# PeihaoChen/RSPNet

Hardware: AMD Instinct MI355X
Metric: clips/sec pretext step (c3d 16x112x112, B=32/GPU) (higher is better)
Workload: dtype f32

## Files before the change

### include/rspnet_hip.h

```cpp
#ifndef RSPNET_HIP_H
#define RSPNET_HIP_H

#include <stddef.h>
#include <stdint.h>

#ifdef __cplusplus
extern "C" {
#endif

#define RSP_OK 0
#define RSP_EINVAL (-1)
#define RSP_EWORKSPACE (-2)
#define RSP_ELAUNCH (-3)
#define RSP_EUNSUPPORTED (-4)

const char* rsp_strerror(int code);
const char* rsp_last_error(void);
const char* rsp_last_conv_kernel(void);
int rsp_version(void);

typedef struct rsp_conv3d_desc {
  int32_t N, Di, Hi, Wi, Cin;
  int32_t Do, Ho, Wo, Cout;
  int32_t kT, kH, kW;
// ... 70 lines not shown
  int32_t kT, kH, kW, sT, sH, sW, pT, pH, pW;
  int32_t in_ld, out_ld, res_ld;
} rsp_pool3d_desc;

int rsp_bn_act_pool_fwd(const rsp_pool3d_desc* d, const float* y, const float* scale_shift, const float* residual,
                        int relu, const float* gate, float* out, void* stream);

int rsp_bn_act_maxpool_applicable(const rsp_pool3d_desc* d);
int rsp_bn_act_maxpool_fwd(const rsp_pool3d_desc* d, const float* y, const float* scale_shift, int relu, const float* gate, float* out,
                           int32_t* argmax, void* stream);

size_t rsp_bn_bwd_workspace(const rsp_pool3d_desc* d);
int rsp_bn_act_pool_bwd(const rsp_pool3d_desc* d, const float* y, const float* residual, const float* dout,
                        const float* gamma, const float* mean_invstd, const float* scale_shift, int relu, float* dy,
                        float* dres, float* dgamma, float* dbeta, int32_t c_valid, const float* gate, const float* dmean,
                        void* workspace, size_t workspace_bytes, void* stream);

int rsp_bn_act_pool_sel_applicable(const rsp_pool3d_desc* d);
int rsp_bn_act_pool_sel_fwd(const rsp_pool3d_desc* d, const float* y, const float* scale_shift, int relu, float* out, float* y_sel,
                            void* stream);
int rsp_bn_act_pool_sel_bwd(const rsp_pool3d_desc* d, const float* y, const float* y_sel, const float* dout, const float* gamma,
                            const float* mean_invstd, const float* scale_shift, int relu, float* dy, float* dgamma, float* dbeta,
                            int32_t c_valid, void* workspace, size_t workspace_bytes, void* stream);

int rsp_bn_act_minmax_fwd(const float* y_max, const float* y_min, int64_t positions, int32_t C, int32_t out_ld,
                          const float* scale_shift, int relu, float* out, void* stream);

size_t rsp_bn_eval_bwd_workspace(const rsp_pool3d_desc* d);
int rsp_bn_eval_act_pool_bwd(const rsp_pool3d_desc* d, const float* y, const float* residual, const float* dout,
                             const float* mean_invstd, const float* scale_shift, int relu, float* dy, float* dres,
                             float* dgamma, float* dbeta, int32_t c_valid, void* workspace, size_t workspace_bytes,
                             void* stream);

int rsp_maxpool3d_fwd(const rsp_pool3d_desc* d, const float* x, float* out, int32_t* argmax, void* stream);
int rsp_maxpool3d_bwd(const rsp_pool3d_desc* d, const float* dout, const int32_t* argmax, float* dx, void* stream);

size_t rsp_gate_fwd_workspace(int32_t N, int32_t P, int32_t C);
int rsp_gate_fwd(const float* x, int32_t N, int32_t P, int32_t C, int32_t in_ld, const float* w, const float* b,
                 float* out, int32_t out_ld, float* mean, float* gate, void* workspace, size_t workspace_bytes,
                 void* stream);
int rsp_bn_gate_sums(const float* y, int32_t N, int32_t P, int32_t C, int32_t y_ld, const float* scale_shift, int relu,
                     float* act, int32_t act_ld, const float* w, const float* b, float* mean, float* gate, void* workspace,
                     size_t workspace_bytes, void* stream);
int rsp_gate_apply(const float* x, int32_t N, int32_t P, int32_t C, int32_t in_ld, const float* gate, float* out, int32_t out_ld,
                   void* stream);
int rsp_gate_bwd_params(const float* y, const float* scale_shift, int relu, const float* dout, int32_t N, int32_t P, int32_t C,
// ... 146 lines not shown
```

### rspnet_amd/_lib.py

```python
from __future__ import annotations

import ctypes as C
import os
from typing import Optional

_HERE = os.path.dirname(os.path.abspath(__file__))
LIB_PATH = os.environ.get("RSPNET_HIP_LIB") or os.path.join(_HERE, "librspnet_hip.so")

c_f32p = C.c_void_p
c_i32p = C.c_void_p
c_stream = C.c_void_p


class ConvDesc(C.Structure):
    _fields_ = [(n, C.c_int32) for n in (
        "N", "Di", "Hi", "Wi", "Cin", "Do", "Ho", "Wo", "Cout", "kT", "kH", "kW", "sT", "sH", "sW",
        "pT", "pH", "pW", "in_ld", "out_ld")]


class PoolDesc(C.Structure):
    _fields_ = [(n, C.c_int32) for n in (
        "N", "Di", "Hi", "Wi", "C", "Do", "Ho", "Wo", "kT", "kH", "kW", "sT", "sH", "sW", "pT", "pH", "pW",
        "in_ld", "out_ld", "res_ld")]

# ... 43 lines not shown
SIGNATURES = {
    "rsp_strerror": (C.c_char_p, [C.c_int]),
    "rsp_last_error": (C.c_char_p, []),
    "rsp_last_conv_kernel": (C.c_char_p, []),
    "rsp_version": (C.c_int, []),
    "rsp_conv3d_packed_fwd_elems": (_sz, [_PD]),
    "rsp_conv3d_pack_fwd": (C.c_int, [_PD, _p, _p, _p]),
    "rsp_conv3d_stat_tiles": (_i32, [_PD]),
    "rsp_conv3d_fwd_workspace": (_sz, [_PD]),
    "rsp_conv3d_fwd": (C.c_int, [_PD, _p, _p, _p, _p, _p, _p, _sz, _p]),
    "rsp_conv3d_stem_pooled_applicable": (C.c_int, [_PD]),
    "rsp_conv3d_stem_pooled_fwd": (C.c_int, [_PD, _p, _p, _p, _p, _p, _p, _p]),
    "rsp_conv3d_dgrad_workspace": (_sz, [_PD]),
    "rsp_conv3d_dgrad": (C.c_int, [_PD, _p, _p, _p, _p, _sz, _p]),
    "rsp_conv3d_packed_dgrad_elems": (_sz, [_PD]),
    "rsp_conv3d_dgrad_packed": (C.c_int, [_PD, _p, _p, _p, _p, _sz, _p]),
    "rsp_conv3d_pack_jobs": (_i32, [_PD, _i32, _i32, _i32, _p, _p, _p, _i32]),
    "rsp_pack_run": (C.c_int, [_p, _i32, _i32, _p]),
    "rsp_conv3d_pack_forget": (None, [_p]),
    "rsp_conv3d_wgrad_workspace": (_sz, [_PD]),
    "rsp_conv3d_rowgeom_bytes": (_sz, [_PD]),
    "rsp_conv3d_rowgeom": (C.c_int, [_PD, _p, _p]),
    "rsp_conv3d_wgrad": (C.c_int, [_PD, _p, _p, _p, _p, _i32, _i32, _p, _p, _sz, _p]),
    "rsp_conv3d_kernel_name": (C.c_char_p, [_PD, C.c_int]),
    "rsp_conv3d_executed_fraction": (C.c_double, [_PD, C.c_int]),
    "rsp_conv3d_set_option": (C.c_int, [C.c_char_p, _i32]),
    "rsp_fastdiv_check": (C.c_int, [C.c_int, C.c_int]),
    "rsp_bn_finalize_workspace": (_sz, [_i32, _i32]),
    "rsp_bn_finalize": (C.c_int, [_p, _i32, _i32, _i32, _i32, _i64, _p, _p, _p, _f, _f, _p, _p, _p, _p, _p, _p, _sz, _p]),
    "rsp_bn_running_update": (C.c_int, [_p, _i32, _i32, _p]),
    "rsp_bn_act_pool_fwd": (C.c_int, [_PP, _p, _p, _p, C.c_int, _p, _p, _p]),
    "rsp_bn_act_maxpool_applicable": (C.c_int, [_PP]),
    "rsp_bn_act_maxpool_fwd": (C.c_int, [_PP, _p, _p, C.c_int, _p, _p, _p, _p]),
    "rsp_bn_bwd_workspace": (_sz, [_PP]),
    "rsp_bn_act_pool_bwd": (C.c_int, [_PP, _p, _p, _p, _p, _p, _p, C.c_int, _p, _p, _p, _p, _i32, _p, _p, _p, _sz, _p]),
    "rsp_bn_act_pool_sel_applicable": (C.c_int, [_PP]),
    "rsp_bn_act_pool_sel_fwd": (C.c_int, [_PP, _p, _p, C.c_int, _p, _p, _p]),
    "rsp_bn_act_pool_sel_bwd": (C.c_int, [_PP, _p, _p, _p, _p, _p, _p, C.c_int, _p, _p, _p, _i32, _p, _sz, _p]),
    "rsp_bn_act_minmax_fwd": (C.c_int, [_p, _p, _i64, _i32, _i32, _p, C.c_int, _p, _p]),
    "rsp_bn_eval_bwd_workspace": (_sz, [_PP]),
    "rsp_bn_eval_act_pool_bwd": (C.c_int, [_PP, _p, _p, _p, _p, _p, C.c_int, _p, _p, _p, _p, _i32, _p, _sz, _p]),
    "rsp_maxpool3d_fwd": (C.c_int, [_PP, _p, _p, _p, _p]),
    "rsp_maxpool3d_bwd": (C.c_int, [_PP, _p, _p, _p, _p]),
    "rsp_gate_fwd_workspace": (_sz, [_i32, _i32, _i32]),
    "rsp_gate_fwd": (C.c_int, [_p, _i32, _i32, _i32, _i32, _p, _p, _p, _i32, _p, _p, _p, _sz, _p]),
    "rsp_bn_gate_sums": (C.c_int, [_p, _i32, _i32, _i32, _i32, _p, C.c_int, _p, _i32, _p, _p, _p, _p, _p, _sz, _p]),
# ... 109 lines not shown
```

### rspnet_amd/csrc/bn_pool.hip

```cpp
#include "common.h"

namespace {

__global__ __launch_bounds__(256) void bn_finalize_stage1(const float* __restrict__ part, int tiles, int C, int ld, int S,
                                                          double* __restrict__ out) {
  __shared__ double red[4][64][2];
  const int c = blockIdx.x * 64 + (threadIdx.x & 63);
  const int rl = threadIdx.x >> 6;
  const int per = (tiles + S - 1) / S;
  const int t0 = blockIdx.y * per, t1 = min(tiles, t0 + per);
  double s = 0.0, ss = 0.0;
  if (c < C)
    for (int t = t0 + rl; t < t1; t += 4) {
      const float2 v = *reinterpret_cast<const float2*>(part + ((long long)t * ld + c) * 2);
      s += (double)v.x;
      ss += (double)v.y;
    }
  red[rl][threadIdx.x & 63][0] = s;
  red[rl][threadIdx.x & 63][1] = ss;
  __syncthreads();
  if (rl == 0 && c < C) {
    const int l = threadIdx.x;
    out[((long long)blockIdx.y * C + c) * 2 + 0] = red[0][l][0] + red[1][l][0] + red[2][l][0] + red[3][l][0];
    out[((long long)blockIdx.y * C + c) * 2 + 1] = red[0][l][1] + red[1][l][1] + red[2][l][1] + red[3][l][1];
// ... 845 lines not shown
      constexpr int NW = MODE == 2 ? 4 : 8;
      long long off[NW];
      window_offsets<NW>(d, off);
      for (; o < o_end; o += stride) {
        const int op = (int)o;
        const int q1 = fastdiv(op, p.dWo), ow = op - q1 * d.Wo;
        const int q2 = fastdiv(q1, p.dHo), oh = q1 - q2 * d.Ho;
        const int n = fastdiv(q2, p.dDo), od = q2 - n * d.Do;
        const long long base = (((long long)n * d.Di + od * d.sT) * d.Hi + oh * d.sH) * d.Wi + ow * d.sW;
        float yv[NW][VEC], r[NW][VEC], g[VEC], best[VEC];
        int bi[VEC];
#pragma unroll
        for (int w = 0; w < NW; ++w) {
          load_vec<VEC>(p.y + (base + off[w]) * d.in_ld + c, yv[w]);
          if (p.res) load_vec<VEC>(p.res + (base + off[w]) * d.res_ld + c, r[w]);
        }
        load_vec<VEC>(p.dout + o * d.out_ld + c, g);
#pragma unroll
        for (int e = 0; e < VEC; ++e) { best[e] = -INFINITY; bi[e] = 0; }
#pragma unroll
        for (int w = 0; w < NW; ++w)
#pragma unroll
          for (int e = 0; e < VEC; ++e) {
            float z = fmaf(yv[w][e], sc[e], sh[e]);
            if (p.res) z += r[w][e];
            const float v = p.relu ? rsp_relu(z) : z;
            if (rsp_max_takes(v, best[e])) { best[e] = v; bi[e] = w; }
          }
#pragma unroll
        for (int w = 0; w < NW; ++w) {
          float ov[VEC], dz[VEC];
#pragma unroll
          for (int e = 0; e < VEC; ++e) {
            dz[e] = (bi[e] == w && !(p.relu && rsp_relu_blocks(best[e]))) ? g[e] : 0.f;
            const float xhat = (yv[w][e] - mean[e]) * invstd[e];
            ov[e] = gam[e] * invstd[e] * (dz[e] - m1[e] - xhat * m2[e]);
          }
          store_vec<VEC>(p.dy + (base + off[w]) * d.in_ld + c, ov);
          if (p.dres) store_vec<VEC>(p.dres + (base + off[w]) * d.res_ld + c, dz);
        }
      }
    }
    return;
  }
  for (; o < o_end; o += stride) {
    float g[VEC];
    load_vec<VEC>(p.dout + o * d.out_ld + c, g);
    if (MODE == 1 || nwin == 1) {
      if (p.gate) gated_grad<VEC>(p, fastdiv(fastdiv(fastdiv((int)o, p.dWo), p.dHo), p.dDo), c, g);
      float yv[VEC], z[VEC], ov[VEC], dz[VEC];
      zval<VEC>(p, o, c, sc, sh, yv, z);
#pragma unroll
      for (int e = 0; e < VEC; ++e) {
        dz[e] = (p.relu && rsp_relu_blocks(z[e])) ? 0.f : g[e];
        const float xhat = (yv[e] - mean[e]) * invstd[e];
        ov[e] = gam[e] * invstd[e] * (dz[e] - m1[e] - xhat * m2[e]);
      }
      store_vec<VEC>(p.dy + o * d.in_ld + c, ov);
      if (p.dres) store_vec<VEC>(p.dres + o * d.res_ld + c, dz);
// ... 424 lines not shown
      (!gate || rsp_aligned16(gate)))
    return rsp_bn_act_maxpool_fwd(d, y, scale_shift, relu, gate, out, nullptr, stream);
  PoolParams p;
  p.d = *d; p.y = y; p.ss = scale_shift; p.res = residual; p.gate = gate; p.out = out; p.relu = relu;
  const bool vec = d->C % 4 == 0 && d->in_ld % 4 == 0 && d->out_ld % 4 == 0 && rsp_aligned16(y) && rsp_aligned16(out) &&
                   rsp_aligned16(scale_shift) && (!residual || (d->res_ld % 4 == 0 && rsp_aligned16(residual))) &&
                   (!gate || rsp_aligned16(gate));
  p.cg = vec ? d->C / 4 : d->C;
  const Layout L = make_layout(d, p.cg, 4);
  RSP_REQUIRE(L.npos < (1ll << 31), "rsp_bn_act_pool_fwd: more than 2^31 - 1 output positions");
  set_layout(p, L);
  RSP_BN_LAUNCH(bn_act_pool_fwd_kernel, vec, bn_mode(d, gate != nullptr), L.grid, (hipStream_t)stream, p);
  return rsp_check_launch("bn_act_pool_fwd_kernel");
}

size_t rsp_bn_bwd_workspace(const rsp_pool3d_desc* d) {
  if (!pool_ok(d, true)) return 0;
  return rsp_align_up((size_t)2048 * d->C * 2 * sizeof(float), 256) + (size_t)d->C * 2 * sizeof(double);
}

static int bn_act_pool_bwd(const rsp_pool3d_desc* d, const float* y, const float* y_sel, const float* residual, const float* dout,
                           const float* gamma, const float* mean_invstd, const float* scale_shift, int relu, float* dy,
                           float* dres, float* dgamma, float* dbeta, int32_t c_valid, const float* gate, const float* dmean,
                           void* workspace, size_t workspace_bytes, void* stream) {
  RSP_REQUIRE(pool_ok(d, true), "rsp_bn_act_pool_bwd: needs disjoint windows (kernel == stride, no padding)");
  RSP_REQUIRE(!gate || (dmean && d->kT * d->kH * d->kW == 1 && d->sT * d->sH * d->sW == 1 && !residual),
              "rsp_bn_act_pool_bwd: a gated unit has a unit window, no residual, and needs dmean");
  RSP_REQUIRE(c_valid > 0 && c_valid <= d->C, "rsp_bn_act_pool_bwd: bad valid channel count");
  RSP_REQUIRE(y && dout && mean_invstd && scale_shift && dy && workspace, "rsp_bn_act_pool_bwd: null pointer");
  if (workspace_bytes < rsp_bn_bwd_workspace(d)) {
    rsp_set_error("rsp_bn_act_pool_bwd: workspace too small");
    return RSP_EWORKSPACE;
  }
  hipStream_t s = (hipStream_t)stream;
  BwdParams p;
  memset(&p, 0, sizeof p);
  p.d = *d; p.y = y; p.res = residual; p.dout = dout; p.gamma = gamma; p.mi = mean_invstd; p.ss = scale_shift;
  p.dy = dy; p.dres = dres; p.relu = relu;
  p.Cv = c_valid;
  p.gate = gate; p.dmean = dmean;
  p.invP = 1.f / (float)((long long)d->Di * d->Hi * d->Wi);
  p.count = (long long)d->N * d->Di * d->Hi * d->Wi;
  const bool vec = d->C % 4 == 0 && d->in_ld % 4 == 0 && d->out_ld % 4 == 0 && rsp_aligned16(y) && rsp_aligned16(dout) &&
                   rsp_aligned16(dy) && rsp_aligned16(scale_shift) && rsp_aligned16(mean_invstd) &&
                   (!gamma || c_valid != d->C || rsp_aligned16(gamma)) &&
                   (!residual || (d->res_ld % 4 == 0 && rsp_aligned16(residual) && (!dres || rsp_aligned16(dres)))) &&
                   (!gate || (rsp_aligned16(gate) && rsp_aligned16(dmean)));
  p.cg = vec ? d->C / 4 : d->C;
  p.partial = reinterpret_cast<float*>(workspace);
  double* sums = reinterpret_cast<double*>(reinterpret_cast<unsigned char*>(workspace) +
                                           rsp_align_up((size_t)2048 * d->C * 2 * sizeof(float), 256));
  p.sums = sums;
  const Layout L = make_layout(d, p.cg, 4);
  RSP_REQUIRE(L.npos < (1ll << 31), "rsp_bn_act_pool_bwd: more than 2^31 - 1 output positions");
  set_layout(p, L);
  p.nblocks = reduce_blocks(d, p.cg);
  dim3 rgrid(p.nblocks, rsp_cdiv(p.cg, 256));
  const int mode = bn_mode(d, gate != nullptr);
  if (y_sel) {
    RSP_REQUIRE(vec && (mode == 2 || mode == 3) && !residual && rsp_aligned16(y_sel),
                "rsp_bn_act_pool_sel_bwd: y_sel needs what rsp_bn_act_pool_sel_fwd needs, and no residual");
    p.ysel = y_sel;
    hipLaunchKernelGGL(bn_bwd_reduce_sel_kernel<4>, rgrid, dim3(256), 0, s, p);
  } else {
    RSP_BN_LAUNCH(bn_bwd_reduce_kernel, vec, mode, rgrid, s, p);
  }
  int rc = rsp_check_launch("bn_bwd_reduce_kernel");
  if (rc != RSP_OK) return rc;
  hipLaunchKernelGGL(bn_bwd_finalize_kernel, dim3(rsp_cdiv(d->C, FIN_CH)), dim3(1024), 0, s, p.partial, p.nblocks, d->C, c_valid, sums,
                     dgamma, dbeta);
  rc = rsp_check_launch("bn_bwd_finalize_kernel");
  if (rc != RSP_OK) return rc;
  const bool exact = d->Di % d->sT == 0 && d->Hi % d->sH == 0 && d->Wi % d->sW == 0 && d->kT * d->kH * d->kW <= 8;
  if (exact) {
    RSP_BN_LAUNCH(bn_bwd_apply_win_kernel, vec, mode, L.grid, s, p);
    return rsp_check_launch("bn_bwd_apply_win_kernel");
  }
  const long long total = (long long)d->N * d->Di * d->Hi * d->Wi * p.cg;
  if (vec) hipLaunchKernelGGL(bn_bwd_apply_kernel<4>, dim3(grid_for(total)), dim3(256), 0, s, p);
  else hipLaunchKernelGGL(bn_bwd_apply_kernel<1>, dim3(grid_for(total)), dim3(256), 0, s, p);
  return rsp_check_launch("bn_bwd_apply_kernel");
}

int rsp_bn_act_pool_bwd(const rsp_pool3d_desc* d, const float* y, const float* residual, const float* dout,
                        const float* gamma, const float* mean_invstd, const float* scale_shift, int relu, float* dy,
                        float* dres, float* dgamma, float* dbeta, int32_t c_valid, const float* gate, const float* dmean,
                        void* workspace, size_t workspace_bytes, void* stream) {
  return bn_act_pool_bwd(d, y, nullptr, residual, dout, gamma, mean_invstd, scale_shift, relu, dy, dres, dgamma, dbeta, c_valid, gate,
                         dmean, workspace, workspace_bytes, stream);
}

int rsp_bn_act_pool_sel_bwd(const rsp_pool3d_desc* d, const float* y, const float* y_sel, const float* dout, const float* gamma,
                            const float* mean_invstd, const float* scale_shift, int relu, float* dy, float* dgamma, float* dbeta,
                            int32_t c_valid, void* workspace, size_t workspace_bytes, void* stream) {
  RSP_REQUIRE(y_sel, "rsp_bn_act_pool_sel_bwd: null pointer");
  return bn_act_pool_bwd(d, y, y_sel, nullptr, dout, gamma, mean_invstd, scale_shift, relu, dy, nullptr, dgamma, dbeta, c_valid, nullptr,
                         nullptr, workspace, workspace_bytes, stream);
}

static int eval_bwd_mode(const rsp_pool3d_desc* d) {
  const int m = bn_mode(d, false);
  if (m == 1) return 1;
  const bool exact = d->Di % d->sT == 0 && d->Hi % d->sH == 0 && d->Wi % d->sW == 0;
  return exact ? m : 0;
}

static long long eval_bwd_npos(const rsp_pool3d_desc* d, int mode) {
  if (mode != 0) return (long long)d->N * d->Do * d->Ho * d->Wo;
  return (long long)d->N * rsp_cdiv(d->Di, d->sT) * rsp_cdiv(d->Hi, d->sH) * rsp_cdiv(d->Wi, d->sW);
}

size_t rsp_bn_eval_bwd_workspace(const rsp_pool3d_desc* d) {
  if (!pool_ok(d, true)) return 0;
  const long long npos = eval_bwd_npos(d, eval_bwd_mode(d));
  const long long rows = npos < EVAL_BWD_MAX_BLOCKS ? npos : EVAL_BWD_MAX_BLOCKS;
  return (size_t)rows * d->C * 2 * sizeof(float);
}

#define RSP_BN_EVAL_LAUNCH_S(V, M, grid, stream, p)                                                                       \
  do {                                                                                                                    \
    if (sums) hipLaunchKernelGGL((bn_eval_bwd_kernel<V, M, true>), grid, dim3(256), 0, stream, p);                        \
// ... 60 lines not shown
```

### rspnet_amd/csrc/conv_stem.h

```cpp
#pragma once
#include "common.h"

bool rsp_conv_desc_ok(const rsp_conv3d_desc* d);
bool rsp_stem_applicable(const rsp_conv3d_desc* d);
int rsp_stem_tiles(const rsp_conv3d_desc* d);
size_t rsp_stem_packed_elems(const rsp_conv3d_desc* d);
int rsp_stem_pack(const rsp_conv3d_desc* d, const float* w_ref, float* w_packed, hipStream_t s);
int rsp_stem_fwd(const rsp_conv3d_desc* d, const float* x, const float* w_packed, const float* bias, float* y,
                 float* stat_partials, hipStream_t s);
const char* rsp_stem_kernel_name(const rsp_conv3d_desc* d);
bool rsp_stem_pooled_applicable(const rsp_conv3d_desc* d);
int rsp_stem_pooled_fwd(const rsp_conv3d_desc* d, const float* x, const float* w_packed, const float* bias, float* y_max, float* y_min,
                        float* stat_partials, hipStream_t s);
void rsp_stem_note_packed(const void* w_packed, bool three_channels);
void rsp_stem_forget_packed(const void* w_packed);
const char* rsp_wgrad_kernel_name(const rsp_conv3d_desc* d);
double rsp_wgrad_executed_fraction(const rsp_conv3d_desc* d);
```

### rspnet_amd/csrc/conv_stem.hip

```cpp
#include "conv_stem.h"

#include <mutex>
#include <unordered_map>

namespace {

struct StemParams {
  const float* __restrict__ x;
  const float* __restrict__ w;
  const float* __restrict__ bias;
  float* __restrict__ y;
  float* __restrict__ stat;
  int N, Di, Hi, Wi, Do, Ho, Wo;
  int kT, kH, kW, sT, sH, sW, pT, pH, pW;
  int Cout, out_ld;
  int tw_shift;
  int HT, WT, WTh, WTL;
  int npix, npix_r;
  int FR;
  int ntaps, nchunks;
  int tiles_h, tiles_w, tiles;
  unsigned x_bytes, w_bytes;
  int wide;
  float* __restrict__ ymax;
// ... 395 lines not shown
      }
      s += __shfl_xor(s, 32);
      ss += __shfl_xor(ss, 32);
      if (h == 0) {
        red[(wave * 64 + col) * 2 + 0] = s;
        red[(wave * 64 + col) * 2 + 1] = ss;
      }
    }
    if (p.stat) {
      __syncthreads();
      if (t < 64 && t < p.Cout) {
        float s = 0.f, ss = 0.f;
#pragma unroll
        for (int w = 0; w < 4; ++w) {
          s += red[(w * 64 + t) * 2 + 0];
          ss += red[(w * 64 + t) * 2 + 1];
        }
        float* o = p.stat + ((long long)tile * p.Cout + t) * 2;
        o[0] = s;
        o[1] = ss;
      }
    }
    cur ^= 1;
  }
}

__global__ void stem_pack_kernel(const float* __restrict__ w, float* __restrict__ out, int Cout, int kT, int kH, int kW,
                                 int ntaps, long long total) {
  for (long long i = blockIdx.x * (long long)blockDim.x + threadIdx.x; i < total; i += (long long)gridDim.x * blockDim.x) {
    const int ci = (int)(i & 3), n = (int)((i >> 2) & 63), tap = (int)(i >> 8);
    float v = 0.f;
    if (tap < ntaps && n < Cout) {
      const int kw = tap % kW, r = tap / kW;
      const int kh = r % kH, kt = r / kH;
      v = w[((((long long)n * 4 + ci) * kT + kt) * kH + kh) * kW + kw];
    }
    out[i] = v;
  }
}

struct StemPlan {
  bool ok;
  int G, TCH, nchunks, tw_shift, HT, WT, WTh, WTL, npix, npix_r, FR, tiles_h, tiles_w;
  bool resident;
  bool wide_ok;
  long long tiles;
// ... 187 lines not shown
}

bool rsp_stem_pooled_applicable(const rsp_conv3d_desc* d) { return stem_pooled_ok(d, stem_plan(d)); }

int rsp_stem_pooled_fwd(const rsp_conv3d_desc* d, const float* x, const float* w_packed, const float* bias, float* y_max, float* y_min,
                        float* stat_partials, hipStream_t stream) {
  const StemPlan pl = stem_plan(d);
  RSP_REQUIRE(stem_pooled_ok(d, pl), "rsp_conv3d_stem_pooled_fwd: descriptor not covered (rsp_conv3d_stem_pooled_applicable)");
  RSP_REQUIRE(rsp_aligned16(x) && rsp_aligned16(w_packed) && rsp_aligned16(y_max) && rsp_aligned16(y_min),
              "rsp_conv3d_stem_pooled_fwd: input, packed weight and both outputs must be 16-byte aligned");
  StemParams p = stem_params(d, pl, x, w_packed, bias, stat_partials);
  p.ymax = y_max; p.ymin = y_min; p.pool_ld = d->Cout;
  if (stem_three_channels(w_packed)) {
    switch (pl.G) {
      case 7: return launch_stem_pooled<7, 3>(p, pl, stream);
      default: return launch_stem_pooled<5, 3>(p, pl, stream);
    }
  }
  switch (pl.G) {
    case 7: return launch_stem_pooled<7, 4>(p, pl, stream);
    default: return launch_stem_pooled<5, 4>(p, pl, stream);
  }
}
```

### rspnet_amd/engine.py

```python
from __future__ import annotations

import contextlib
import os
from dataclasses import dataclass, field
from typing import Dict, List, NamedTuple, Optional, Tuple, Union

import torch
from torch import nn

from . import ops as _ops
from .ops import ConvGeom, PoolGeom

Triple = Tuple[int, int, int]


@dataclass
class ConvBN:
    conv: nn.Module
    bn: nn.Module
    src: int
    dst: int
    k: Triple
    s: Triple = (1, 1, 1)
    p: Triple = (0, 0, 0)
# ... 143 lines not shown

class _CatConv:
    weight: torch.Tensor = None


def _adjacent_cat(ts):
    t0 = ts[0]
    if not all(t.is_contiguous() and t.shape[1:] == t0.shape[1:] and t.dtype == t0.dtype for t in ts):
        return None
    end = t0.data_ptr() + t0.numel() * t0.element_size()
    for t in ts[1:]:
        if t.data_ptr() != end or t.untyped_storage().data_ptr() != t0.untyped_storage().data_ptr():
            return None
        end += t.numel() * t.element_size()
    shape = (sum(t.shape[0] for t in ts),) + tuple(t0.shape[1:])
    stride = tuple(t0.stride())
    return torch.as_strided(t0, shape, stride, t0.storage_offset())


INPUT_CHANNEL_PAD = 4
GATE_BWD_FUSED = not os.environ.get("RSP_NO_GATE_BWD_FUSION")
STEM_POOLED = not os.environ.get("RSP_NO_STEM_POOLED")
BN_BWD_SEL = not os.environ.get("RSP_NO_BN_BWD_SEL")


class VirtualStem:

    def __init__(self, node):
        self.conv = node.conv
        w = node.conv.weight
        Cout, cin, kT, kH, kW = w.shape
        assert cin == 3 and kW == 7 and node.s[2] == 2 and node.p[2] == 3
        self.holders, self.idx, self.src, self.dst = [], [], [], []
        co = torch.arange(Cout).view(Cout, 1, 1, 1, 1)
        c4 = torch.arange(4).view(1, 4, 1, 1, 1)
        kt = torch.arange(kT).view(1, 1, kT, 1, 1)
        kh = torch.arange(kH).view(1, 1, 1, kH, 1)
        j = torch.arange(6).view(1, 1, 1, 1, 6)
        for off in (3, 1):
            r = 4 * j + c4 - off
            valid = ((r >= 0) & (r < 21)).expand(Cout, 4, kT, kH, 6)
            real = ((((co * 3 + r % 3) * kT + kt) * kH + kh) * 7 + torch.div(r, 3, rounding_mode="floor")).expand(Cout, 4, kT, kH, 6)
            idx = torch.where(valid, real, torch.full_like(real, w.numel())).reshape(-1)
            flat_valid = valid.reshape(-1).nonzero().view(-1)
            self.idx.append(idx.to(w.device))
            self.src.append(flat_valid.to(w.device))
# ... 482 lines not shown

    def take_grad(self, node, C):
        return _view(self.dslots[node.into[0]], node.into, C) if node.into is not None else self.dslots.pop(node.dst)

    def issued(self, ni):
        if self.hook is not None:
            self.hook(ni, self.branches.grads_ready)

    def input_grad(self, src, cg, dy, conv):
        if src != self.plan.input_slot or self.want_input_grad:
            self.add_grad(src, self.be.conv_dgrad_packed(cg, dy, self.packed.get_dgrad(conv, cg)))

    def convbn(self, node, ni, key=None):
        key = ni if key is None else key
        sv = self.ctx.saved.pop(key)
        if isinstance(sv, _SavedVStem):
            return self.convbn_virtual(node, sv, ni)
        if sv.gate is not None:
            return self.convbn_gated(node, sv, ni)
        if sv.eval_mode:
            return self.convbn_eval(node, sv, ni)
        bn, grad_of = node.bn, self.grad_of
        dout = self.take_grad(node, sv.cg.Cout)
        sel = {} if sv.y_sel is None else {"y_sel": sv.y_sel}
        dy, dres = self.be.bn_act_pool_bwd(sv.pg, sv.y, sv.res, dout, bn.weight.data, sv.mi, sv.ss, node.relu,
                                           node.residual is not None, grad_of(bn.weight), grad_of(bn.bias), **sel)
        self.convbn_tail(node, sv, ni, dy, dres, True)

    def convbn_virtual(self, node, sv, ni):
        be, grad_of, vs, cg = self.be, self.grad_of, sv.vs, sv.cg
        assert node.src == self.plan.input_slot and not self.want_input_grad, "a virtual-pixel stem reads the clip: no input gradient"
        dout = self.dslots.pop(node.dst)
        bn = node.bn
        dy, _ = be.bn_act_pool_bwd(sv.pg, sv.y, None, dout, bn.weight.data, sv.mi, sv.ss, node.relu, False, grad_of(bn.weight), grad_of(bn.bias))
        gw = grad_of(node.conv.weight)
        if gw is not None:
            N, do, ho, Wo, Cp = dy.shape
            dyv = dy.view(N, do, ho, Wo // 2, 2 * Cp)
            gflat = gw.view(-1)
            gflat.zero_()
            for c, xc in enumerate((sv.x_e, sv.x_o)):
                gv = torch.empty_like(vs.holders[c].weight)
                be.conv_wgrad(cg, xc, dyv[..., c * Cp:(c + 1) * Cp], gv)
                gflat.index_add_(0, vs.dst[c], gv.view(-1).index_select(0, vs.src[c]))
        self.issued(ni)

    def convbn_gated(self, node, sv, ni):
        bn, grad_of, sg = node.bn, self.grad_of, sv.gate
        gnode = self.plan.nodes[sg.at]
        dout = self.take_grad(gnode, sv.cg.Cout)
# ... 99 lines not shown
```

### rspnet_amd/ops.py

```python
from __future__ import annotations

import collections
import contextlib
import ctypes as C
import functools
from dataclasses import dataclass
from typing import Optional, Tuple

import torch

from . import _lib


@dataclass(frozen=True)
class ConvGeom:
    N: int
    Di: int
    Hi: int
    Wi: int
    Cin: int
    Cout: int
    k: Tuple[int, int, int]
    s: Tuple[int, int, int]
    p: Tuple[int, int, int]
# ... 58 lines not shown
@functools.lru_cache(maxsize=4096)
def executed_fraction(g: "ConvGeom", which: int) -> float:
    d = g.desc()
    return float(_lib.load().rsp_conv3d_executed_fraction(C.byref(d), which))


@functools.lru_cache(maxsize=8192)
def _pack_signature(g: "ConvGeom", which: int, cout_src: int, cin_src: int):
    lib = _lib.load()
    d = g.desc()
    buf = (_lib.PackJob * 64)()
    cnt = lib.rsp_conv3d_pack_jobs(C.byref(d), which, cout_src, cin_src, C.c_void_p(1 << 20), C.c_void_p(1 << 30), buf, 64)
    lib.rsp_conv3d_pack_forget(C.c_void_p(1 << 30))
    if cnt < 0:
        _lib.check(cnt, "rsp_conv3d_pack_jobs")
    n = (lib.rsp_conv3d_packed_dgrad_elems if which else lib.rsp_conv3d_packed_fwd_elems)(C.byref(d))
    return (int(n), bytes(buf)[:cnt * C.sizeof(_lib.PackJob)])


@functools.lru_cache(maxsize=4096)
def _stem_pooled_ok(g: "ConvGeom") -> bool:
    d = g.desc()
    return bool(_lib.load().rsp_conv3d_stem_pooled_applicable(C.byref(d)))


@functools.lru_cache(maxsize=4096)
def _pool_plan(pg: "PoolGeom", in_ld, out_ld, res_ld):
    lib = _lib.load()
    d = pg.desc(in_ld=in_ld, out_ld=out_ld, res_ld=res_ld)
    ref = C.byref(d)
    return d, ref, lib.rsp_bn_bwd_workspace(ref), pg.out_dims


def _ptr(t: Optional[torch.Tensor]):
    return None if t is None else C.c_void_p(t.data_ptr())


_raw_stream = getattr(torch._C, "_cuda_getCurrentRawStream", None)
_get_device = getattr(torch._C, "_cuda_getDevice", None)


def _stream():
    if _raw_stream is not None and _get_device is not None:
        return C.c_void_p(_raw_stream(_get_device()))
    return C.c_void_p(torch.cuda.current_stream().cuda_stream)

# ... 322 lines not shown
                        want_dres: bool, dgamma_out, dbeta_out, dy_out=None, y_sel=None):
        in_ld = _rows_ld(y, "y")
        d, dref, wsb, _ = _pool_plan(pg, in_ld, _rows_ld(dout, "dout"), None if residual is None else _rows_ld(residual, "residual"))
        dy = _dy_target(y, in_ld, dy_out)
        dres = torch.empty_like(y) if want_dres else None
        ws = self._workspace(y.device, wsb)
        c_valid = pg.C if gamma is None else int(gamma.shape[0])
        e0 = self._ev()
        n_in = y.numel()
        if y_sel is not None:
            if residual is not None or want_dres:
                raise _lib.RspError("bn_act_pool_bwd: y_sel with a residual")
            _lib.check(self.lib.rsp_bn_act_pool_sel_bwd(dref, _ptr(y), _ptr(_chk(y_sel, "y_sel")), _ptr(dout), _ptr(gamma), _ptr(mean_invstd),
                                                        _ptr(scale_shift), int(relu), _ptr(dy), _ptr(dgamma_out), _ptr(dbeta_out), c_valid,
                                                        _ptr(ws), wsb, _stream()), "rsp_bn_act_pool_sel_bwd")
            self._log_hbm("bn_bwd(reduce+apply)", 4 * (y_sel.numel() + 2 * dout.numel() + 2 * n_in), e0)
            return dy, dres
        _lib.check(self.lib.rsp_bn_act_pool_bwd(dref, _ptr(y), _ptr(residual), _ptr(dout), _ptr(gamma),
                                                _ptr(mean_invstd), _ptr(scale_shift), int(relu), _ptr(dy), _ptr(dres),
                                                _ptr(dgamma_out), _ptr(dbeta_out), c_valid, None, None, _ptr(ws), wsb, _stream()),
                   "rsp_bn_act_pool_bwd")
        self._log_hbm("bn_bwd(reduce+apply)", 4 * (2 * (n_in * (1 if residual is None else 2) + dout.numel()) + n_in * (2 if want_dres else 1)), e0)
        return dy, dres

    def bn_eval_act_pool_bwd(self, pg: PoolGeom, y, residual, dout, mean_invstd, scale_shift, relu: bool, want_dres: bool,
                             dgamma_out, dbeta_out, dy_out=None):
        in_ld = _rows_ld(y, "y")
        d, dref, _, _ = _pool_plan(pg, in_ld, _rows_ld(dout, "dout"), None if residual is None else _rows_ld(residual, "residual"))
        dy = _dy_target(y, in_ld, dy_out)
        if want_dres and residual is None:
            raise _lib.RspError("want_dres without a residual")
        dres = torch.empty(y.shape, dtype=torch.float32, device=y.device) if want_dres else None
        if want_dres and d.res_ld != pg.C:
            raise _lib.RspError("residual: a residual whose gradient is wanted must be contiguous")
        sums = dgamma_out is not None or dbeta_out is not None
        c_valid = pg.C
        for v in (dgamma_out, dbeta_out):
            if v is not None:
                c_valid = int(v.shape[0])
        wsb = int(self.lib.rsp_bn_eval_bwd_workspace(dref)) if sums else 0
        ws = self._workspace(y.device, wsb) if sums else None
        e0 = self._ev()
        _lib.check(self.lib.rsp_bn_eval_act_pool_bwd(dref, _ptr(y), _ptr(residual), _ptr(dout), _ptr(mean_invstd), _ptr(scale_shift),
                                                     int(relu), _ptr(dy), _ptr(dres), _ptr(dgamma_out), _ptr(dbeta_out), c_valid,
                                                     _ptr(ws), wsb, _stream()), "rsp_bn_eval_act_pool_bwd")
        n_in = y.numel()
# ... 532 lines not shown
```

Baseline: 357.2.

## Fuse stem BN/ReLU/maxpool backward apply into the stem weight-gradient kernel

Adds a fused stem backward kernel. It recomputes the BN+ReLU+2x2 maxpool input gradient in registers from y and dout and feeds it straight into MFMA-based weight-gradient accumulation against the input halo staged in LDS. The first-layer dy tensor is never written to or read back from HBM. The BN reduction pass still runs separately, and a small reduce kernel sums the per-block partials. In exchange there is a more specialised code path with strict applicability checks and a recompute of the BN backward maths.

```diff
diff --git a/include/rspnet_hip.h b/include/rspnet_hip.h
--- a/include/rspnet_hip.h
+++ b/include/rspnet_hip.h
@@ -116,6 +116,13 @@
 int rsp_bn_act_pool_sel_bwd(const rsp_pool3d_desc* d, const float* y, const float* y_sel, const float* dout, const float* gamma,
                             const float* mean_invstd, const float* scale_shift, int relu, float* dy, float* dgamma, float* dbeta,
                             int32_t c_valid, void* workspace, size_t workspace_bytes, void* stream);
+
+size_t rsp_conv3d_stem_bn_wgrad_workspace(const rsp_conv3d_desc* d, const rsp_pool3d_desc* pd);
+int rsp_conv3d_stem_bn_wgrad(const rsp_conv3d_desc* d, const rsp_pool3d_desc* pd, const float* x, const float* y, const float* y_sel,
+                             const float* residual, const float* gate, const float* dout, const float* gamma,
+                             const float* mean_invstd, const float* scale_shift, int relu, float* dw_ref, int32_t cout_valid,
+                             int32_t cin_valid, float* dgamma, float* dbeta, int32_t c_valid, void* workspace,
+                             size_t workspace_bytes, void* stream);
 
 int rsp_bn_act_minmax_fwd(const float* y_max, const float* y_min, int64_t positions, int32_t C, int32_t out_ld,
                           const float* scale_shift, int relu, float* out, void* stream);
diff --git a/rspnet_amd/_lib.py b/rspnet_amd/_lib.py
--- a/rspnet_amd/_lib.py
+++ b/rspnet_amd/_lib.py
@@ -89,6 +89,8 @@
     "rsp_conv3d_rowgeom_bytes": (_sz, [_PD]),
     "rsp_conv3d_rowgeom": (C.c_int, [_PD, _p, _p]),
     "rsp_conv3d_wgrad": (C.c_int, [_PD, _p, _p, _p, _p, _i32, _i32, _p, _p, _sz, _p]),
+    "rsp_conv3d_stem_bn_wgrad_workspace": (_sz, [_PD, _PP]),
+    "rsp_conv3d_stem_bn_wgrad": (C.c_int, [_PD, _PP, _p, _p, _p, _p, _p, _p, _p, _p, _p, C.c_int, _p, _i32, _i32, _p, _p, _i32, _p, _sz, _p]),
     "rsp_conv3d_kernel_name": (C.c_char_p, [_PD, C.c_int]),
     "rsp_conv3d_executed_fraction": (C.c_double, [_PD, C.c_int]),
     "rsp_conv3d_set_option": (C.c_int, [C.c_char_p, _i32]),
diff --git a/rspnet_amd/csrc/bn_bwd_math.h b/rspnet_amd/csrc/bn_bwd_math.h
--- /dev/null
+++ b/rspnet_amd/csrc/bn_bwd_math.h
@@ -0,0 +1,17 @@
+#pragma once
+#include "common.h"
+
+__device__ __forceinline__ float rsp_bn_bwd_z(float y, float sc, float sh) { return fmaf(y, sc, sh); }
+
+__device__ __forceinline__ void rsp_bn_bwd_scan(float v, int w, float& best, int& bi) {
+  if (rsp_max_takes(v, best)) { best = v; bi = w; }
+}
+
+__device__ __forceinline__ float rsp_bn_bwd_dz(int w, int bi, float best, bool relu, float g) {
+  return (bi == w && !(relu && rsp_relu_blocks(best))) ? g : 0.f;
+}
+
+__device__ __forceinline__ float rsp_bn_bwd_dy(float y, float dz, float mean, float invstd, float gam, float m1, float m2) {
+  const float xhat = (y - mean) * invstd;
+  return gam * invstd * (dz - m1 - xhat * m2);
+}
diff --git a/rspnet_amd/csrc/bn_pool.hip b/rspnet_amd/csrc/bn_pool.hip
--- a/rspnet_amd/csrc/bn_pool.hip
+++ b/rspnet_amd/csrc/bn_pool.hip
@@ -1,4 +1,6 @@
 #include "common.h"
+#include "bn_bwd_math.h"
+#include "conv_stem.h"
 
 namespace {
 
@@ -891,19 +893,18 @@
         for (int w = 0; w < NW; ++w)
 #pragma unroll
           for (int e = 0; e < VEC; ++e) {
-            float z = fmaf(yv[w][e], sc[e], sh[e]);
+            float z = rsp_bn_bwd_z(yv[w][e], sc[e], sh[e]);
             if (p.res) z += r[w][e];
             const float v = p.relu ? rsp_relu(z) : z;
-            if (rsp_max_takes(v, best[e])) { best[e] = v; bi[e] = w; }
+            rsp_bn_bwd_scan(v, w, best[e], bi[e]);
           }
 #pragma unroll
         for (int w = 0; w < NW; ++w) {
           float ov[VEC], dz[VEC];
 #pragma unroll
           for (int e = 0; e < VEC; ++e) {
-            dz[e] = (bi[e] == w && !(p.relu && rsp_relu_blocks(best[e]))) ? g[e] : 0.f;
-            const float xhat = (yv[w][e] - mean[e]) * invstd[e];
-            ov[e] = gam[e] * invstd[e] * (dz[e] - m1[e] - xhat * m2[e]);
+            dz[e] = rsp_bn_bwd_dz(w, bi[e], best[e], p.relu != 0, g[e]);
+            ov[e] = rsp_bn_bwd_dy(yv[w][e], dz[e], mean[e], invstd[e], gam[e], m1[e], m2[e]);
           }
           store_vec<VEC>(p.dy + (base + off[w]) * d.in_ld + c, ov);
           if (p.dres) store_vec<VEC>(p.dres + (base + off[w]) * d.res_ld + c, dz);
@@ -1374,12 +1375,12 @@
 static int bn_act_pool_bwd(const rsp_pool3d_desc* d, const float* y, const float* y_sel, const float* residual, const float* dout,
                            const float* gamma, const float* mean_invstd, const float* scale_shift, int relu, float* dy,
                            float* dres, float* dgamma, float* dbeta, int32_t c_valid, const float* gate, const float* dmean,
-                           void* workspace, size_t workspace_bytes, void* stream) {
+                           void* workspace, size_t workspace_bytes, void* stream, const double** sums_only = nullptr) {
   RSP_REQUIRE(pool_ok(d, true), "rsp_bn_act_pool_bwd: needs disjoint windows (kernel == stride, no padding)");
   RSP_REQUIRE(!gate || (dmean && d->kT * d->kH * d->kW == 1 && d->sT * d->sH * d->sW == 1 && !residual),
               "rsp_bn_act_pool_bwd: a gated unit has a unit window, no residual, and needs dmean");
   RSP_REQUIRE(c_valid > 0 && c_valid <= d->C, "rsp_bn_act_pool_bwd: bad valid channel count");
-  RSP_REQUIRE(y && dout && mean_invstd && scale_shift && dy && workspace, "rsp_bn_act_pool_bwd: null pointer");
+  RSP_REQUIRE(y && dout && mean_invstd && scale_shift && (dy || sums_only) && workspace, "rsp_bn_act_pool_bwd: null pointer");
   if (workspace_bytes < rsp_bn_bwd_workspace(d)) {
     rsp_set_error("rsp_bn_act_pool_bwd: workspace too small");
     return RSP_EWORKSPACE;
@@ -1423,6 +1424,10 @@
                      dgamma, dbeta);
   rc = rsp_check_launch("bn_bwd_finalize_kernel");
   if (rc != RSP_OK) return rc;
+  if (sums_only) {
+    *sums_only = sums;
+    return RSP_OK;
+  }
   const bool exact = d->Di % d->sT == 0 && d->Hi % d->sH == 0 && d->Wi % d->sW == 0 && d->kT * d->kH * d->kW <= 8;
   if (exact) {
     RSP_BN_LAUNCH(bn_bwd_apply_win_kernel, vec, mode, L.grid, s, p);
@@ -1449,6 +1454,17 @@
   return bn_act_pool_bwd(d, y, y_sel, nullptr, dout, gamma, mean_invstd, scale_shift, relu, dy, nullptr, dgamma, dbeta, c_valid, nullptr,
                          nullptr, workspace, workspace_bytes, stream);
 }
+
+}
+
+int rsp_bn_bwd_sums(const rsp_pool3d_desc* d, const float* y, const float* y_sel, const float* dout, const float* gamma,
+                    const float* mean_invstd, const float* scale_shift, int relu, float* dgamma, float* dbeta, int32_t c_valid,
+                    void* workspace, size_t workspace_bytes, void* stream, const double** sums) {
+  return bn_act_pool_bwd(d, y, y_sel, nullptr, dout, gamma, mean_invstd, scale_shift, relu, nullptr, nullptr, dgamma, dbeta, c_valid, nullptr,
+                         nullptr, workspace, workspace_bytes, stream, sums);
+}
+
+extern "C" {
 
 static int eval_bwd_mode(const rsp_pool3d_desc* d) {
   const int m = bn_mode(d, false);
diff --git a/rspnet_amd/csrc/conv_stem.h b/rspnet_amd/csrc/conv_stem.h
--- a/rspnet_amd/csrc/conv_stem.h
+++ b/rspnet_amd/csrc/conv_stem.h
@@ -14,5 +14,8 @@
                         float* stat_partials, hipStream_t s);
 void rsp_stem_note_packed(const void* w_packed, bool three_channels);
 void rsp_stem_forget_packed(const void* w_packed);
+int rsp_bn_bwd_sums(const rsp_pool3d_desc* d, const float* y, const float* y_sel, const float* dout, const float* gamma,
+                    const float* mean_invstd, const float* scale_shift, int relu, float* dgamma, float* dbeta, int32_t c_valid,
+                    void* workspace, size_t workspace_bytes, void* stream, const double** sums);
 const char* rsp_wgrad_kernel_name(const rsp_conv3d_desc* d);
 double rsp_wgrad_executed_fraction(const rsp_conv3d_desc* d);
diff --git a/rspnet_amd/csrc/conv_stem.hip b/rspnet_amd/csrc/conv_stem.hip
--- a/rspnet_amd/csrc/conv_stem.hip
+++ b/rspnet_amd/csrc/conv_stem.hip
@@ -1,4 +1,5 @@
 #include "conv_stem.h"
+#include "bn_bwd_math.h"
 
 #include <mutex>
 #include <unordered_map>
@@ -441,6 +442,234 @@
       }
     }
     cur ^= 1;
+  }
+}
+
+struct StemBwdParams {
+  StemParams s;
+  const float* __restrict__ yv;
+  const float* __restrict__ dout;
+  const float* __restrict__ ss;
+  const float* __restrict__ mi;
+  const float* __restrict__ gamma;
+  const double* __restrict__ sums;
+  float* __restrict__ partial;
+  int dout_ld, Cv;
+  long long count;
+};
+
+__global__ __launch_bounds__(256, 2) void stem_bn_wgrad_kernel(const StemBwdParams q) {
+  const StemParams& p = q.s;
+  typedef __attribute__((address_space(3))) void* lptr_t;
+  extern __shared__ __attribute__((aligned(16))) unsigned char smem_raw[];
+  const int hsz = p.kT * p.npix_r * 4;
+  float* halo = reinterpret_cast<float*>(smem_raw);
+
+  const int t = threadIdx.x;
+  const int lane = t & 63;
+  const int wave = __builtin_amdgcn_readfirstlane(t >> 6);
+  const int l32 = lane & 31, h = lane >> 5;
+
+  __amdgpu_buffer_rsrc_t rsrc_x = __builtin_amdgcn_make_buffer_rsrc(const_cast<float*>(p.x), 0, (int)p.x_bytes, 0x00020000);
+  int hyy[4], wxp[4];
+#pragma unroll
+  for (int i = 0; i < 4; ++i) {
+    const int k = i * 256 + t;
+    hyy[i] = -(1 << 20);
+    wxp[i] = 0;
+    if (k < p.npix) {
+      hyy[i] = k / p.WTL;
+      wxp[i] = k - hyy[i] * p.WTL;
+    }
+  }
+  auto issue_halo = [&](int tile, int buf) {
+    const int wb = tile % p.tiles_w;
+    int q0 = tile / p.tiles_w;
+    const int hb = q0 % p.tiles_h;
+    q0 /= p.tiles_h;
+    const int to = q0 % p.Do, n = q0 / p.Do;
+    const int hi0 = hb * 8 - p.pH, wi0 = wb * 16 - p.pW;
+    unsigned hrel[4];
+#pragma unroll
+    for (int i = 0; i < 4; ++i) {
+      const int hi = hi0 + hyy[i], wi = wi0 + wxp[i];
+      hrel[i] = ((unsigned)hi < (unsigned)p.Hi && (unsigned)wi < (unsigned)p.Wi) ? (unsigned)((hi * p.Wi + wi) * 16) : 0xffffffffu;
+    }
+    for (int f = 0; f < p.kT; ++f) {
+      const int ti = to - p.pT + f;
+      const bool okf = (unsigned)ti < (unsigned)p.Di;
+      const unsigned fbase = (unsigned)(((long long)(n * p.Di + (okf ? ti : 0)) * p.Hi * p.Wi) * 16);
+#pragma unroll
+      for (int i = 0; i < 4; ++i) {
+        if (i * 256 + wave * 64 < p.npix_r) {
+          const unsigned off = (okf & (hrel[i] != 0xffffffffu)) ? fbase + hrel[i] : 0xffffffffu;
+          float* dst = halo + buf * hsz + (f * p.npix_r + i * 256 + wave * 64) * 4;
+          __builtin_amdgcn_raw_ptr_buffer_load_lds(rsrc_x, (lptr_t)dst, 16, off, 0, 0, 0);
+        }
+      }
+    }
+  };
+
+  float sc[2], sh[2], mean[2], invstd[2], gam[2], m1[2], m2[2];
+  bool cok[2];
+  const double invn = 1.0 / (double)q.count;
+#pragma unroll
+  for (int j = 0; j < 2; ++j) {
+    const int c = 32 * j + l32;
+    cok[j] = c < p.Cout;
+    sc[j] = sh[j] = mean[j] = invstd[j] = gam[j] = m1[j] = m2[j] = 0.f;
+    if (cok[j]) {
+      sc[j] = q.ss[c];
+      sh[j] = q.ss[p.Cout + c];
+      mean[j] = q.mi[c];
+      invstd[j] = q.mi[p.Cout + c];
+      gam[j] = c < q.Cv ? (q.gamma ? q.gamma[c] : 1.f) : 0.f;
+      m1[j] = (float)(q.sums[2 * c] * invn);
+      m2[j] = (float)(q.sums[2 * c + 1] * invn);
+    }
+  }
+  int boff[3];
+#pragma unroll
+  for (int b = 0; b < 3; ++b) {
+    const int n = 32 * b + l32;
+    int off = 0;
+    if (n < 3 * p.ntaps) {
+      const int tap = n / 3, ch = n - 3 * tap;
+      const int kw = tap % p.kW, r = tap / p.kW;
+      const int kh = r % p.kH, kt = r / p.kH;
+      off = ((kt * p.npix_r) + kh * p.WTL + kw) * 16 + ch * 4;
+    }
+    boff[b] = off + (2 * wave * p.WTL + 4 * h) * 16;
+  }
+  const int erow = p.WTL * 16;
+
+  const int HoP = p.Ho >> 1, WoP = p.Wo >> 1;
+  auto load_patch = [&](int tile, float (&yv)[2][16], float (&g)[2][4]) {
+    const int wb = tile % p.tiles_w;
+    int q0 = tile / p.tiles_w;
+    const int hb = q0 % p.tiles_h;
+    q0 /= p.tiles_h;
+    const float* yb = q.yv + (((long long)q0 * p.Ho + hb * 8 + 2 * wave) * p.Wo + wb * 16 + 4 * h) * p.out_ld;
+    const float* gb = q.dout + (((long long)q0 * HoP + hb * 4 + wave) * WoP + wb * 8 + 2 * h) * q.dout_ld;
+#pragma unroll
+    for (int j = 0; j < 2; ++j) {
+      const int c = cok[j] ? 32 * j + l32 : 0;
+#pragma unroll
+      for (int e = 0; e < 16; ++e) {
+        const int ro = (e >> 3) * p.Wo + 8 * ((e >> 2) & 1) + (e & 3);
+        yv[j][e] = yb[(long long)ro * p.out_ld + c];
+      }
+#pragma unroll
+      for (int k = 0; k < 4; ++k) g[j][k] = gb[(long long)((k >> 1) * 4 + (k & 1)) * q.dout_ld + c];
+    }
+  };
+
+  floatx16 acc[2][3];
+#pragma unroll
+  for (int j = 0; j < 2; ++j)
+#pragma unroll
+    for (int b = 0; b < 3; ++b)
+#pragma unroll
+      for (int e = 0; e < 16; ++e) acc[j][b][e] = 0.f;
+
+  float yn[2][16], gn[2][4];
+  int cur = 0;
+  if ((int)blockIdx.x < p.tiles) {
+    load_patch(blockIdx.x, yn, gn);
+    issue_halo(blockIdx.x, 0);
+  }
+  for (int tile = blockIdx.x; tile < p.tiles; tile += gridDim.x) {
+    __syncthreads();
+    const int next = tile + gridDim.x;
+    floatx16 a[2];
+#pragma unroll
+    for (int j = 0; j < 2; ++j)
+#pragma unroll
+      for (int k = 0; k < 4; ++k) {
+        const int el[4] = {2 * k, 2 * k + 1, 2 * k + 8, 2 * k + 9};
+        float yw[4], best = -INFINITY;
+        int bi = 0;
+        const float g = cok[j] ? gn[j][k] : 0.f;
+#pragma unroll
+        for (int w = 0; w < 4; ++w) yw[w] = cok[j] ? yn[j][el[w]] : 0.f;
+#pragma unroll
+        for (int w = 0; w < 4; ++w) rsp_bn_bwd_scan(rsp_relu(rsp_bn_bwd_z(yw[w], sc[j], sh[j])), w, best, bi);
+#pragma unroll
+        for (int w = 0; w < 4; ++w)
+          a[j][el[w]] = rsp_bn_bwd_dy(yw[w], rsp_bn_bwd_dz(w, bi, best, true, g), mean[j], invstd[j], gam[j], m1[j], m2[j]);
+      }
+    const char* bp = reinterpret_cast<const char*>(halo + cur * hsz);
+    auto bval = [&](int e, int b) {
+      return *reinterpret_cast<const float*>(bp + boff[b] + (e >> 3) * erow + (8 * ((e >> 2) & 1) + (e & 3)) * 16);
+    };
+#pragma unroll
+    for (int e = 0; e < 8; ++e) {
+      float bv[3];
+#pragma unroll
+      for (int b = 0; b < 3; ++b) bv[b] = bval(e, b);
+#pragma unroll
+      for (int b = 0; b < 3; ++b)
+#pragma unroll
+        for (int j = 0; j < 2; ++j) acc[j][b] = __builtin_amdgcn_mfma_f32_32x32x2f32(a[j][e], bv[b], acc[j][b], 0, 0, 0);
+    }
+    float bq[8][3];
+#pragma unroll
+    for (int e = 0; e < 8; ++e)
+#pragma unroll
+      for (int b = 0; b < 3; ++b) bq[e][b] = bval(8 + e, b);
+    if (next < p.tiles) {
+      load_patch(next, yn, gn);
+      issue_halo(next, cur ^ 1);
+    }
+#pragma unroll
+    for (int e = 0; e < 8; ++e)
+#pragma unroll
+      for (int b = 0; b < 3; ++b)
+#pragma unroll
+        for (int j = 0; j < 2; ++j) acc[j][b] = __builtin_amdgcn_mfma_f32_32x32x2f32(a[j][8 + e], bq[e][b], acc[j][b], 0, 0, 0);
+    cur ^= 1;
+  }
+
+  float* stage = halo;
+  float* out = q.partial + (long long)blockIdx.x * (64 * 96);
+#pragma unroll
+  for (int j = 0; j < 2; ++j)
+#pragma unroll
+    for (int b = 0; b < 3; ++b) {
+      __syncthreads();
+      if (wave > 0) {
+#pragma unroll
+        for (int e = 0; e < 16; ++e) stage[((wave - 1) * 16 + e) * 64 + lane] = acc[j][b][e];
+      }
+      __syncthreads();
+      if (wave == 0) {
+#pragma unroll
+        for (int e = 0; e < 16; ++e) {
+          float v = acc[j][b][e];
+#pragma unroll
+          for (int w = 0; w < 3; ++w) v += stage[(w * 16 + e) * 64 + lane];
+          const int co = 32 * j + 8 * (e >> 2) + 4 * h + (e & 3);
+          out[co * 96 + 32 * b + l32] = v;
+        }
+      }
+    }
+}
+
+__global__ __launch_bounds__(256) void stem_bn_wgrad_reduce_kernel(const float* __restrict__ partial, int nparts, float* __restrict__ dw,
+                                                                   int ntaps) {
+  __shared__ float red[8][32];
+  const int nl = threadIdx.x & 31, pl = threadIdx.x >> 5;
+  const int co = blockIdx.y, n = 32 * blockIdx.x + nl;
+  float s = 0.f;
+  for (int g = pl; g < nparts; g += 8) s += partial[((long long)g * 64 + co) * 96 + n];
+  red[pl][nl] = s;
+  __syncthreads();
+  if (pl == 0 && n < 3 * ntaps) {
+    float v = red[0][nl];
+#pragma unroll
+    for (int k = 1; k < 8; ++k) v += red[k][nl];
+    const int tap = n / 3, ch = n - 3 * tap;
+    dw[((long long)co * 3 + ch) * ntaps + tap] = v;
   }
 }
 
@@ -674,3 +903,66 @@
     default: return launch_stem_pooled<5, 4>(p, pl, stream);
   }
 }
+
+static bool stem_bn_wgrad_ok(const rsp_conv3d_desc* d, const rsp_pool3d_desc* pd, const StemPlan& pl) {
+  if (!rsp_conv_desc_ok(d) || !pl.ok || !pl.resident || pl.tw_shift != 4) return false;
+  if (d->sT != 1 || d->sH != 1 || d->sW != 1 || d->kT * d->kH * d->kW * 3 > 96) return false;
+  if (d->Ho % 8 || d->Wo % 16) return false;
+  if (pd->N != d->N || pd->Di != d->Do || pd->Hi != d->Ho || pd->Wi != d->Wo || pd->C != d->Cout || pd->in_ld != d->out_ld) return false;
+  if (pd->kT != 1 || pd->kH != 2 || pd->kW != 2 || pd->sT != 1 || pd->sH != 2 || pd->sW != 2 || pd->pT || pd->pH || pd->pW) return false;
+  if (pd->Do != d->Do || pd->Ho != d->Ho / 2 || pd->Wo != d->Wo / 2 || pd->out_ld < pd->C) return false;
+  return true;
+}
+
+static long long stem_bn_wgrad_grid(const StemPlan& pl) { return pl.tiles < 512 ? pl.tiles : 512; }
+
+extern "C" size_t rsp_conv3d_stem_bn_wgrad_workspace(const rsp_conv3d_desc* d, const rsp_pool3d_desc* pd) {
+  if (!d || !pd) return 0;
+  const StemPlan pl = stem_plan(d);
+  if (!stem_bn_wgrad_ok(d, pd, pl)) return 0;
+  const size_t bn = rsp_bn_bwd_workspace(pd);
+  if (!bn) return 0;
+  return rsp_align_up(bn, 256) + (size_t)stem_bn_wgrad_grid(pl) * 64 * 96 * sizeof(float);
+}
+
+extern "C" int rsp_conv3d_stem_bn_wgrad(const rsp_conv3d_desc* d, const rsp_pool3d_desc* pd, const float* x, const float* y,
+                                        const float* y_sel, const float* residual, const float* gate, const float* dout,
+                                        const float* gamma, const float* mean_invstd, const float* scale_shift, int relu, float* dw_ref,
+                                        int32_t cout_valid, int32_t cin_valid, float* dgamma, float* dbeta, int32_t c_valid,
+                                        void* workspace, size_t workspace_bytes, void* stream) {
+  RSP_REQUIRE(d && pd, "rsp_conv3d_stem_bn_wgrad: null descriptor");
+  const StemPlan pl = stem_plan(d);
+  if (!stem_bn_wgrad_ok(d, pd, pl) || residual || gate || !relu || cin_valid != 3) {
+    rsp_set_error("rsp_conv3d_stem_bn_wgrad: not covered (resident stride-1 stem of three real input channels on 8x16 patches that tile "
+                  "the frame, ReLU, MaxPool(1,2,2), no residual, no gate)");
+    return RSP_EUNSUPPORTED;
+  }
+  RSP_REQUIRE(x && y && dout && mean_invstd && scale_shift && dw_ref && workspace, "rsp_conv3d_stem_bn_wgrad: null pointer");
+  RSP_REQUIRE(rsp_aligned16(x) && rsp_aligned16(workspace), "rsp_conv3d_stem_bn_wgrad: input and workspace must be 16-byte aligned");
+  RSP_REQUIRE(cout_valid > 0 && cout_valid <= d->Cout, "rsp_conv3d_stem_bn_wgrad: bad valid channel counts");
+  RSP_REQUIRE(c_valid > 0 && c_valid <= d->Cout, "rsp_conv3d_stem_bn_wgrad: bad valid channel count");
+  if (workspace_bytes < rsp_conv3d_stem_bn_wgrad_workspace(d, pd)) {
+    rsp_set_error("rsp_conv3d_stem_bn_wgrad: workspace too small");
+    return RSP_EWORKSPACE;
+  }
+  hipStream_t s = (hipStream_t)stream;
+  const size_t bn = rsp_bn_bwd_workspace(pd);
+  const double* sums = nullptr;
+  int rc = rsp_bn_bwd_sums(pd, y, y_sel, dout, gamma, mean_invstd, scale_shift, relu, dgamma, dbeta, c_valid, workspace, bn, stream, &sums);
+  if (rc != RSP_OK) return rc;
+  StemBwdParams q;
+  memset(&q, 0, sizeof q);
+  q.s = stem_params(d, pl, x, nullptr, nullptr, nullptr);
+  q.yv = y; q.dout = dout; q.ss = scale_shift; q.mi = mean_invstd; q.gamma = gamma; q.sums = sums;
+  q.partial = reinterpret_cast<float*>(reinterpret_cast<unsigned char*>(workspace) + rsp_align_up(bn, 256));
+  q.dout_ld = pd->out_ld; q.Cv = c_valid;
+  q.count = (long long)d->N * d->Do * d->Ho * d->Wo;
+  const long long grid = stem_bn_wgrad_grid(pl);
+  size_t lds = (size_t)2 * d->kT * pl.npix_r * 16;
+  if (lds < 3 * 16 * 64 * sizeof(float)) lds = 3 * 16 * 64 * sizeof(float);
+  rc = rsp_launch_lds<stem_bn_wgrad_kernel>(dim3((unsigned)grid), lds, 80 * 1024, s, std::tie(q), "stem_bn_wgrad_kernel");
+  if (rc != RSP_OK) return rc;
+  hipLaunchKernelGGL(stem_bn_wgrad_reduce_kernel, dim3(3, (unsigned)cout_valid), dim3(256), 0, s, q.partial, (int)grid, dw_ref,
+                     d->kT * d->kH * d->kW);
+  return rsp_check_launch("stem_bn_wgrad_reduce_kernel");
+}
diff --git a/rspnet_amd/engine.py b/rspnet_amd/engine.py
--- a/rspnet_amd/engine.py
+++ b/rspnet_amd/engine.py
@@ -189,6 +189,7 @@
 GATE_BWD_FUSED = not os.environ.get("RSP_NO_GATE_BWD_FUSION")
 STEM_POOLED = not os.environ.get("RSP_NO_STEM_POOLED")
 BN_BWD_SEL = not os.environ.get("RSP_NO_BN_BWD_SEL")
+STEM_BWD_FUSED = not os.environ.get("RSP_NO_STEM_BWD_FUSED")
 
 
 class VirtualStem:
@@ -717,10 +718,31 @@
             return self.convbn_eval(node, sv, ni)
         bn, grad_of = node.bn, self.grad_of
         dout = self.take_grad(node, sv.cg.Cout)
+        if self.stem_fused(node, sv, ni, dout):
+            return
         sel = {} if sv.y_sel is None else {"y_sel": sv.y_sel}
         dy, dres = self.be.bn_act_pool_bwd(sv.pg, sv.y, sv.res, dout, bn.weight.data, sv.mi, sv.ss, node.relu,
                                            node.residual is not None, grad_of(bn.weight), grad_of(bn.bias), **sel)
         self.convbn_tail(node, sv, ni, dy, dres, True)
+
+    def stem_fused(self, node, sv, ni, dout):
+        be, grad_of = self.be, self.grad_of
+        if not (STEM_BWD_FUSED and hasattr(be, "stem_bn_wgrad")):
+            return False
+        gw = grad_of(node.conv.weight)
+        if (node.src != self.plan.input_slot or self.want_input_grad or node.residual is not None or sv.res is not None or
+                not node.relu or gw is None):
+            return False
+        bn = node.bn
+        if not be.stem_bn_wgrad(sv.cg, sv.pg, sv.x, sv.y, dout, bn.weight.data, sv.mi, sv.ss, node.relu, gw, grad_of(bn.weight),
+                                grad_of(bn.bias), y_sel=sv.y_sel):
+            return False
+        bias = getattr(node.conv, "bias", None)
+        gb = grad_of(bias) if bias is not None else None
+        if gb is not None:
+            gb.zero_()
+        self.issued(ni)
+        return True
 
     def convbn_virtual(self, node, sv, ni):
         be, grad_of, vs, cg = self.be, self.grad_of, sv.vs, sv.cg
diff --git a/rspnet_amd/ops.py b/rspnet_amd/ops.py
--- a/rspnet_amd/ops.py
+++ b/rspnet_amd/ops.py
@@ -104,6 +104,13 @@
 def _stem_pooled_ok(g: "ConvGeom") -> bool:
     d = g.desc()
     return bool(_lib.load().rsp_conv3d_stem_pooled_applicable(C.byref(d)))
+
+
+@functools.lru_cache(maxsize=4096)
+def _stem_bn_wgrad_workspace(g: "ConvGeom", pg: "PoolGeom", in_ld, out_ld, dout_ld) -> int:
+    d = g.desc(in_ld=in_ld, out_ld=out_ld)
+    pd = pg.desc(in_ld=out_ld, out_ld=dout_ld)
+    return int(_lib.load().rsp_conv3d_stem_bn_wgrad_workspace(C.byref(d), C.byref(pd)))
 
 
 @functools.lru_cache(maxsize=4096)
@@ -472,6 +479,30 @@
                    "rsp_bn_act_pool_bwd")
         self._log_hbm("bn_bwd(reduce+apply)", 4 * (2 * (n_in * (1 if residual is None else 2) + dout.numel()) + n_in * (2 if want_dres else 1)), e0)
         return dy, dres
+
+    def stem_bn_wgrad(self, g: ConvGeom, pg: PoolGeom, x, y, dout, gamma, mean_invstd, scale_shift, relu: bool, dw_out, dgamma_out,
+                      dbeta_out, y_sel=None) -> bool:
+        _chk(x, "x")
+        _chk(dw_out, "dw_out")
+        in_ld = _rows_ld(y, "y")
+        d, dref, _, _, _, _, _, _ = _conv_plan(g, None, None if in_ld == g.Cout else in_ld)
+        pd, pref, _, _ = _pool_plan(pg, in_ld, _rows_ld(dout, "dout"), None)
+        wsb = _stem_bn_wgrad_workspace(g, pg, d.in_ld, d.out_ld, pd.out_ld)
+        if not wsb or not relu or dw_out.shape[1] != 3 or dw_out.shape[0] > g.Cout or x.data_ptr() % 16:
+            return False
+        if y_sel is not None:
+            _chk(y_sel, "y_sel")
+        ws = self._workspace(x.device, wsb)
+        c_valid = pg.C if gamma is None else int(gamma.shape[0])
+        e0 = self._ev()
+        _lib.check(self.lib.rsp_conv3d_stem_bn_wgrad(dref, pref, _ptr(x), _ptr(y), _ptr(y_sel), None, None, _ptr(dout), _ptr(gamma),
+                                                     _ptr(mean_invstd), _ptr(scale_shift), int(relu), _ptr(dw_out), dw_out.shape[0],
+                                                     dw_out.shape[1], _ptr(dgamma_out), _ptr(dbeta_out), c_valid, _ptr(ws), wsb, _stream()),
+                   "rsp_conv3d_stem_bn_wgrad")
+        n_sel = y.numel() if y_sel is None else y_sel.numel()
+        self._log_hbm("bn_bwd(reduce)+stem_wgrad", 4 * (n_sel + 2 * dout.numel() + y.numel() + x.numel()), e0)
+        self._log("conv_wgrad", g, e0, "stem_bn_wgrad_kernel")
+        return True
 
     def bn_eval_act_pool_bwd(self, pg: PoolGeom, y, residual, dout, mean_invstd, scale_shift, relu: bool, want_dres: bool,
                              dgamma_out, dbeta_out, dy_out=None):
```

Result: no change. 360.1, median of 6 (+0.8%).
